# thomasdeppisch/eMagLS

Hardware: AMD Instinct MI355X
Metric: eMagLS filter sets/s (N=4, 2702 dirs, 512 taps) (higher is better)
Workload: dtype f64; 1 GPU; BASELINE config 3: getEMagLsFilters em32 r=4.2cm N=4 complex-SH, 2702 dirs, 512 taps, 48 kHz; one filter set per step, inputs resident in HBM; dirs=2702, taps=512, sim_order=19, bins=512, k_cut=43, designs_resident_per_gpu=128, designs_per_batch=32, batches_in_flight=4, distinct_hrir_sets_resident=20, parallelism=independent jobs per GPU, one RCCL gather

## Files before the change

### emagls_amd/csrc/fft.hip

```cpp
#include "kernels.hpp"
#include "lds_fft.hpp"
#include "wave_fft.hpp"

namespace emagls {

__global__ void twiddle_kernel(int nfft, cplx* __restrict__ tw, size_t bstride) {
    tw = boff(tw, bstride);
    int j = blockIdx.x * blockDim.x + threadIdx.x;
    if (j >= nfft) return;
    double s, c;
    sincos(-2.0 * kPi * (double)j / (double)nfft, &s, &c);
    if (j == 0) { c = 1.0; s = 0.0; }
    if (2 * j == nfft) { c = -1.0; s = 0.0; }
    if (4 * j == nfft) { c = 0.0; s = -1.0; }
    if (4 * j == 3 * nfft) { c = 0.0; s = 1.0; }
    tw[j] = mk(c, s);
}

__global__ void __launch_bounds__(256) hrir_dirsum_kernel(const double* __restrict__ hL, const double* __restrict__ hR,
                                                          int64_t L, int64_t D, int chunk, double* __restrict__ partial, size_t bstride) {
    hL = boff(hL, bstride); hR = boff(hR, bstride); partial = boff(partial, bstride);
    const int e = blockIdx.y;
    const double* h = e ? hR : hL;
    const int64_t d0 = (int64_t)blockIdx.x * chunk;
// ... 225 lines not shown
                double* row = Habs + ((int64_t)e * na + (kb - kabs0)) * ldD + d0;
                if (nt == HF_TD) {
#pragma unroll
                    for (int t = 0; t < HF_TD; t += 2) *reinterpret_cast<double2*>(row + t) = make_double2(habs[s][e][t], habs[s][e][t + 1]);
                } else {
#pragma unroll
                    for (int t = 0; t < HF_TD; ++t) if (t < nt) row[t] = habs[s][e][t];
                }
            }
        }
    }
}

constexpr int HW_TD = 8;
constexpr int HW_STRIDE = WF_BUF + 1;
__global__ void __launch_bounds__(64 * HW_TD) hrir_fft_wave_kernel(const double* __restrict__ hL, const double* __restrict__ hR,
                                                                   int64_t L, int64_t D, const int64_t* __restrict__ didx,
                                                                   const cplx* __restrict__ tw, const double* __restrict__ grpd,
                                                                   int mode, int n_c, int kabs0, cplx* __restrict__ Hc,
                                                                   double* __restrict__ Habs, int64_t ldD, double* __restrict__ HcT, int ldT,
                                                                   size_t bstride) {
    hL = boff(hL, bstride); hR = boff(hR, bstride); didx = boff(didx, bstride); tw = boff(tw, bstride); grpd = boff(grpd, bstride); Hc = boff(Hc, bstride); Habs = boff(Habs, bstride);
    HcT = boff(HcT, bstride);
    extern __shared__ __attribute__((aligned(16))) char smem[];
    constexpr int P = WF_N / 2 + 1;
    cplx* tables = reinterpret_cast<cplx*>(smem);
    cplx* bufs = tables + WF_TABLES;
    const int tid = threadIdx.x, w = tid >> 6, l = tid & 63;
    wave_fft_tables(tables, tw, tid, 64 * HW_TD);
    __syncthreads();
    const int64_t d0 = (int64_t)blockIdx.x * HW_TD;
    const int nt = (int)min((int64_t)HW_TD, D - d0);
    cplx* tb = bufs + (size_t)w * HW_STRIDE;
    if (w < nt) {
        const int64_t d = d0 + w;
        const int64_t dsrc = didx ? didx[d] : d;
        const double* pl = hL + dsrc * L;
        const double* pr = hR + dsrc * L;
        cplx v[16];
        const bool upper_zero = mode == 0 && L <= WF_N / 2;
        if (mode == 0) {
#pragma unroll
            for (int n1 = 0; n1 < 16; ++n1) {
                const int n = 64 * n1 + l;
                v[n1] = (n < L && (n1 < 8 || !upper_zero)) ? mk(pl[n], pr[n]) : mk(0.0, 0.0);
            }
        } else {
            const int sL = (int)round(grpd[0]), sR = (int)round(grpd[1]);
#pragma unroll
            for (int n1 = 0; n1 < 16; ++n1) {
                const int n = 64 * n1 + l;
                int nl = (n + sL) % WF_N; if (nl < 0) nl += WF_N;
                int nr = (n + sR) % WF_N; if (nr < 0) nr += WF_N;
                v[n1] = mk(nl < L ? pl[nl] : 0.0, nr < L ? pr[nr] : 0.0);
            }
        }
        bool nzL = false, nzR = false;
#pragma unroll
        for (int n1 = 0; n1 < 16; ++n1) { nzL |= v[n1].x != 0.0; nzR |= v[n1].y != 0.0; }
        const bool liveL = __any(nzL), liveR = __any(nzR);
        if (upper_zero) wave_fft1024<true>(v, tb, tables, l); else wave_fft1024<false>(v, tb, tables, l);
        wave_fft_store_natural(v, tb, l);
        wave_lds_fence();
        const cplx* phs = reinterpret_cast<const cplx*>(grpd + 2);
#pragma unroll
        for (int s = 0; s < 9; ++s) {
            const int kb = l + 64 * s;
            if (kb < P) {
                const cplx z = tb[wf_slot(kb)], zc = conj(tb[wf_slot((WF_N - kb) & (WF_N - 1))]);
                cplx HLv = mk(0.5 * (z.x + zc.x), 0.5 * (z.y + zc.y));
                cplx HRv = mk(0.5 * (z.y - zc.y), -0.5 * (z.x - zc.x));
                if (mode == 0) {
                    HLv = HLv * phs[kb];
                    HRv = HRv * phs[P + kb];
                }
                if (!liveL) HLv = mk(0.0, 0.0);
                if (!liveR) HRv = mk(0.0, 0.0);
                if (kb < n_c) {
                    Hc[((int64_t)0 * n_c + kb) * ldD + d] = HLv;
                    Hc[((int64_t)1 * n_c + kb) * ldD + d] = HRv;
                    if (HcT) {
                        double* rowT = HcT + d * ldT;
                        *reinterpret_cast<cplx*>(rowT + 2 * kb) = HLv;
                        *reinterpret_cast<cplx*>(rowT + 2 * (n_c + kb)) = HRv;
                    }
                }
                const double nl2 = norm2(HLv), nr2 = norm2(HRv);
                tb[wf_slot(kb)] = mk(nl2 > 0.0 ? nl2 * fast_rsqrt(nl2) : 0.0, nr2 > 0.0 ? nr2 * fast_rsqrt(nr2) : 0.0);
            }
        }
    }
    __syncthreads();
    const int64_t na = P - kabs0;
    const int t = tid & (HW_TD - 1);
    if (t < nt) {
        const double* src = reinterpret_cast<const double*>(bufs + (size_t)t * HW_STRIDE);
        for (int idx = tid >> 3; idx < 2 * (P - kabs0); idx += 64) {
            const int e = idx >= P - kabs0, kr = idx - e * (P - kabs0);
            Habs[((int64_t)e * na + kr) * ldD + d0 + t] = src[2 * wf_slot(kr + kabs0) + e];
        }
    }
}

__global__ void __launch_bounds__(512) real_fft_gather_kernel(const double* __restrict__ x, int64_t L, int64_t ncols,
                                                              const int64_t* __restrict__ colidx, int nfft, int log2n,
                                                              int TP, const cplx* __restrict__ tw,
                                                              cplx* __restrict__ out, int64_t ldo, int64_t inner,
                                                              int64_t ld_inner) {
    extern __shared__ __attribute__((aligned(16))) char smem[];
    cplx* tws = reinterpret_cast<cplx*>(smem);
    cplx* buf = tws + nfft / 2;
    const int P = nfft / 2 + 1;
    const int64_t p0 = (int64_t)blockIdx.x * TP;
    const int64_t npairs = (ncols + 1) / 2;
    const int nt = (int)min((int64_t)TP, npairs - p0);
// ... 270 lines not shown
                     int64_t ldD, hipStream_t st, double* HcT, int ldT) {
    if (!is_pow2(nfft)) {
        int td = HD_TD;
        while (td > 1 && (size_t)td * 2 * L * 8 > 48 * 1024) td >>= 1;
        if ((size_t)td * 2 * L * 8 > 64 * 1024) throw Error(2, "HRIR DFT: more than 4096 taps is not supported");
        hrir_dft_kernel<<<bgrid((unsigned)ceil_div(D, td)), 256, (size_t)td * 2 * L * 8, st>>>(hL, hR, L, D, didx, nfft, (const cplx*)tw, grpd, mode, n_c, kabs0,
                                                                                                (cplx*)Hc, Habs, ldD, HcT, ldT, td, batch_ctx().stride);
        KERNEL_CHECK();
        return;
    }
    const int log2n = ilog2(nfft);
    const int P = nfft / 2 + 1;
    if (P > HF_MAXS * 512) throw Error(2, "HRIR FFT: nfft above 2048 is not supported");
    if (nfft == WF_N && L <= WF_N && sw_on<Sw::HRIR_FFT_WAVE>()) {
        const size_t smw = sizeof(cplx) * (WF_TABLES + (size_t)HW_TD * HW_STRIDE);
        static PerDeviceOnce wave_once;
        if (wave_once.first())
            HIP_CHECK(hipFuncSetAttribute((const void*)hrir_fft_wave_kernel, hipFuncAttributeMaxDynamicSharedMemorySize, 160 * 1024));
        hrir_fft_wave_kernel<<<bgrid((unsigned)ceil_div(D, HW_TD)), 64 * HW_TD, smw, st>>>(hL, hR, L, D, didx, (const cplx*)tw, grpd, mode, n_c, kabs0,
                                                                                      (cplx*)Hc, Habs, ldD, HcT, ldT, batch_ctx().stride);
        KERNEL_CHECK();
        return;
    }
    size_t budget = (nfft >= 2048 ? 110 : 83) * 1024;
    if (const int kb = sw_int<Sw::HRIR_FFT_LDS_KB>()) budget = (size_t)kb * 1024;
    const size_t shared = (size_t)2 * P * 16 + 2 * HF_TD * sizeof(int);
    int TS = HF_TD;
    while (TS > 1 && (size_t)TS * nfft * 16 + shared > budget) TS >>= 1;
    const size_t sm = (size_t)TS * nfft * 16 + shared;
    static PerDeviceOnce attr_once;
    if (attr_once.first()) {
        HIP_CHECK(hipFuncSetAttribute((const void*)hrir_fft_kernel<8>, hipFuncAttributeMaxDynamicSharedMemorySize, 160 * 1024));
        HIP_CHECK(hipFuncSetAttribute((const void*)hrir_fft_kernel<4>, hipFuncAttributeMaxDynamicSharedMemorySize, 160 * 1024));
        HIP_CHECK(hipFuncSetAttribute((const void*)hrir_fft_kernel<2>, hipFuncAttributeMaxDynamicSharedMemorySize, 160 * 1024));
        HIP_CHECK(hipFuncSetAttribute((const void*)hrir_fft_kernel<1>, hipFuncAttributeMaxDynamicSharedMemorySize, 160 * 1024));
// ... 64 lines not shown
```

### emagls_amd/csrc/sweep_reg.hip

```cpp
#include "device_mem.hpp"
#include "persist_common.hpp"
#include "synth_common.hpp"

#include <algorithm>
#include <map>
#include <mutex>

namespace emagls {

namespace {

constexpr int RG_MLD = 36;

constexpr int DPP_ROR4 = 0x124, DPP_ROR8 = 0x128;
__device__ __forceinline__ int rg_slot_set(int i, int x) { return i < 4 ? 0 : i < 8 ? 1 : x >> 1; }
__device__ __forceinline__ int rg_slot_unit(int i, int x) { return i < 8 ? 4 * (i & 3) + x : 16 + (x & 1); }

template <int NUL>
__device__ __forceinline__ void rg_contract(const cplx (&E)[NUL], const cplx (&O)[NUL], const cplx (&ts)[2], int lane, bool slot8, double* wp) {
    static_assert(NUL == 9, "quad layout of 18 units");
    const int x = lane & 3;
    double ar[2], ai[2];
#pragma unroll
    for (int s = 0; s < 2; ++s) { ar[s] = (x & 1) ? ts[s].y : ts[s].x; ai[s] = (x & 1) ? -ts[s].x : ts[s].y; }
// ... 70 lines not shown
        if (n + 2 >= nord_pad) break;
        request(n + 4, b0, b1);
        pass(c0, c1);
        lds_wait2(b0, b1, pb[GS - 1]);
    }
}

__device__ __forceinline__ int launder(int v) { asm volatile("" : "+v"(v)); return v; }

#define RG_GLOBAL(T, p) ((T __attribute__((address_space(1)))*)(p))
typedef const double __attribute__((address_space(1)))* gcd_t;
typedef const cplx __attribute__((address_space(1)))* gcc_t;
typedef u64 __attribute__((address_space(1)))* gu64_t;
typedef unsigned u32x4_t __attribute__((ext_vector_type(4)));
__device__ __forceinline__ cplx ldg(gcc_t p) { return mk(p->x, p->y); }
__device__ __forceinline__ u64 gll_load(gu64_t p) { return __hip_atomic_load(p, __ATOMIC_RELAXED, __HIP_MEMORY_SCOPE_AGENT); }
__device__ __forceinline__ void gll_put(gu64_t dst, u64 word, bool local) {
    if (local) __hip_atomic_store(dst, word, __ATOMIC_RELAXED, __HIP_MEMORY_SCOPE_WORKGROUP);
    else __hip_atomic_store(dst, word, __ATOMIC_RELAXED, __HIP_MEMORY_SCOPE_AGENT);
}
__device__ __forceinline__ void gll_load16_async(u32x4_t& out, gu64_t p) { asm volatile("global_load_dwordx4 %0, %1, off sc1" : "=v"(out) : "v"(p) : "memory"); }

constexpr int RG_POLL = 12;
__device__ __forceinline__ void rg_wait_loads(u32x4_t (&g)[RG_POLL]) {
    asm volatile("s_waitcnt vmcnt(0)" : "+v"(g[0]), "+v"(g[1]), "+v"(g[2]), "+v"(g[3]), "+v"(g[4]), "+v"(g[5]), "+v"(g[6]), "+v"(g[7]), "+v"(g[8]), "+v"(g[9]),
                 "+v"(g[10]), "+v"(g[11]) :: "memory");
}
constexpr int RG_NUL = 9;
constexpr int RG_NEX = 4 * PS_CMAX;
constexpr int RG_SVC = 256;

template <int NUL, int NW>
__global__ void __launch_bounds__(64 * NW) __attribute__((amdgpu_waves_per_eu(3))) sweep_reg_kernel(const HalfSweepArgs* __restrict__ args, int n, int nWG, int spread, int prio) {
    constexpr int NT = 64 * NW, DPW = 32 * NW;
    constexpr int NU2 = 2 * NUL;
    constexpr int NVW = 8 * NU2;
    constexpr int GA = (NUL + 1) / 2, GB = NUL - GA;
    static_assert(GB >= 1 && NW % 2 == 0 && NT >= RG_SVC, "layout");
    extern __shared__ __attribute__((aligned(16))) char dyn[];
    cplx* ring = reinterpret_cast<cplx*>(dyn);
    cplx* ms = ring + 2 * SY_NORD;
    cplx* WE = ms + PS_CMAX * RG_MLD;
    cplx* WO = WE + 2 * NU2;
    double* vt = reinterpret_cast<double*>(WO + 2 * NU2);
    double* wpart = vt + 2 * RG_NEX;
    double* xs = wpart + NW * NVW;
    __shared__ int s_abort, s_local;

    int design, member;
    if (spread) {
        design = (int)blockIdx.x / nWG;
        member = (int)blockIdx.x - design * nWG;
    } else {
        const int xcd = blockIdx.x & 7, rest = blockIdx.x >> 3;
        const int sub = rest / nWG;
        member = rest - sub * nWG;
        design = xcd + 8 * sub;
    }
    if (design >= n) return;
    if (prio) __builtin_amdgcn_s_setprio(3);
    const HalfSweepArgs& a = args[design];
    const int tid = threadIdx.x;
    const int C = a.C, P = a.P, D = a.D, kfirst = a.kfirst, kabs0 = a.kabs0;
    const int64_t ldH = a.ldH;
    const int nord_pad = a.nord_pad;
    const gcd_t Habs = RG_GLOBAL(const double, a.Habs);
    const gcc_t Mw = RG_GLOBAL(const cplx, a.Mw);
    const gcc_t bsc = RG_GLOBAL(const cplx, a.bsc);
    const gcd_t Winit = RG_GLOBAL(const double, a.Winit);
    cplx __attribute__((address_space(1)))* const Uout = RG_GLOBAL(cplx, a.U);
    long long* const timing = a.timing;
    int* const abort_flag = a.abort_flag;
    const long long wait_ticks = a.wait_ticks;
    const int* smap = a.smap;
    const int npr = smap[32], nsg = smap[33], nun = npr + nsg;
    const gu64_t part_ll = RG_GLOBAL(u64, a.ll);
    const gu64_t xcc_ll = part_ll + (size_t)2 * nWG * RG_NEX * 2;
    if (tid == 0) { s_abort = 0; s_local = 0; }
    const int d0 = member * DPW;
// ... 20 lines not shown
                synth_zen(a.mic_zen ? a.mic_zen[jm] : 1.5707963267948966, sm, cm);
                v = synth_x2(s ? sd[1] : sd[0], s ? cd[1] : cd[0], sm, cm, (s ? daz[1] : daz[0]) - a.mic_azi[jm]);
            }
            xs[i * NT + tid] = v;
        }
    }
    __syncthreads();

    if (tid < nord_pad) {
        ring[(kfirst & 1) * SY_NORD + tid] = ldg(bsc + (int64_t)kfirst * nord_pad + tid);
        const int k1 = kfirst + 1 < P ? kfirst + 1 : P - 1;
        ring[((kfirst + 1) & 1) * SY_NORD + tid] = ldg(bsc + (int64_t)k1 * nord_pad + tid);
    }
    constexpr int NLM = 4;
    cplx mReg[NLM];
    auto fetch_m = [&](int kbm, int t) __attribute__((always_inline)) {
        const int r = t >> 3, c0 = (t & 7) * 4;
        const gcc_t M = Mw + (int64_t)kbm * C * C + r * C + c0;
#pragma unroll
        for (int i = 0; i < NLM; ++i) mReg[i] = ldg(M + i);
    };
    auto stage_m = [&](int t) __attribute__((always_inline)) {
        const int r = t >> 3, c0 = (t & 7) * 4;
#pragma unroll
        for (int i = 0; i < NLM; ++i) ms[r * RG_MLD + c0 + i] = (r < C && c0 + i < C) ? mReg[i] : mk(0, 0);
    };
    double hCur[2], hNext[2] = {0.0, 0.0};
    auto fetch_h = [&](int kb, double (&h)[2], int t) __attribute__((always_inline)) {
        const int kbg = (kb < P ? kb : P - 1) - kabs0;
        const gcd_t He = Habs + ((int64_t)((t >> 1) & 1) * (P - kabs0) + kbg) * ldH;
#pragma unroll
        for (int s = 0; s < 2; ++s) h[s] = He[dir_of(t, s) < D ? dir_of(t, s) : D - 1];
    };
    fetch_h(kfirst, hCur, tid);
    if (tid < RG_SVC) { fetch_m(kfirst, tid); stage_m(tid); }

    if (tid < 64) {
        const int lane = tid;
        const unsigned xcc = read_xcc_id();
        const unsigned tag0 = 0x58434300u;
        if (lane == 0) gll_put(xcc_ll + member, ((u64)tag0 << 32) | xcc, false);
        bool alive = true, same = true;
        for (int base = 0; base < nWG && alive; base += 64) {
            u64 w = 0;
            alive = ll_wait([&] {
                if (base + lane >= nWG) return true;
                w = gll_load(xcc_ll + base + lane);
                return ll_ok(w, tag0);
            }, abort_flag, wait_ticks);
            same = same && __builtin_amdgcn_ballot_w64(base + lane < nWG && (unsigned)w != xcc) == 0;
// ... 24 lines not shown
            const double* xcol = xs + launder(tid);
            synth_units<0, GA, NUL, NT>(xcol, E, O, bs, nord_pad);
            __builtin_amdgcn_sched_barrier(0);
            if (slot8) synth_units<GA, GB, NUL, NT>(xcol, E, O, bs, nord_pad);
            else synth_units<GA, GB - 1, NUL, NT>(xcol, E, O, bs, nord_pad);
            __builtin_amdgcn_sched_barrier(0);
        }
        RSTAMP(0);
        if (launder(tid) < RG_SVC) {
            const int t = launder(tid);
            const int j = t & (RG_NEX - 1), half = t >> 7;
            if (first) {
                vt[t] = half == 0 ? Winit[j] : 0.0;
            } else {
                const unsigned tag = (unsigned)(kb - 1);
                const gu64_t src = part_ll + ((size_t)((kb - 1) & 1) * nWG * RG_NEX + j) * 2;
                double sum = 0.0;
                const bool alive = ll_wait([&] {
                    bool ok = true;
                    double s = 0.0;
                    for (int base = half; base < nWG; base += 2 * RG_POLL) {
                        u32x4_t g[RG_POLL];
#pragma unroll
                        for (int i = 0; i < RG_POLL; ++i) {
                            const int w = base + 2 * i < nWG ? base + 2 * i : half;
                            gll_load16_async(g[i], src + (size_t)w * RG_NEX * 2);
                        }
                        rg_wait_loads(g);
#pragma unroll
                        for (int i = 0; i < RG_POLL; ++i) {
                            ok = ok && g[i].y == tag && g[i].w == tag;
                            if (base + 2 * i < nWG) s += __hiloint2double((int)g[i].z, (int)g[i].x);
                        }
                    }
                    sum = s;
                    return ok;
                }, abort_flag, wait_ticks);
                vt[t] = sum;
                if (!alive && (t & 63) == 0) s_abort = 1;
            }
        }
// ... 2 lines not shown
        if (s_abort) break;
        if (launder(tid) < RG_SVC) {
            const int t = launder(tid);
            const int part = t & 3, pair = t >> 2, e = pair >> 5, c = pair & 31;
            const cplx* vc = reinterpret_cast<const cplx*>(vt) + e * PS_CMAX;
            cplx acc = mk(0, 0);
            if (first) {
                if (part == 0) acc = vc[c];
            } else {
#pragma unroll
                for (int i = 0; i < PS_CMAX / 4; ++i)
                    cfma(acc, vc[part + 4 * i] + vc[RG_NEX / 2 + part + 4 * i], conj(ms[(part + 4 * i) * RG_MLD + c]));
            }
            acc = group_sum<4>(acc);
            const cplx other = shfl_xor_c(acc, 4);
            if (part == 0 && c < C) {
                if (c < 2 * npr) {
                    if ((c & 1) == 0) { WE[e * NU2 + (c >> 1)] = acc + other; WO[e * NU2 + (c >> 1)] = acc - other; }
                } else {
                    WE[e * NU2 + npr + (c - 2 * npr)] = acc; WO[e * NU2 + npr + (c - 2 * npr)] = acc;
                }
                if (member == 0 && !first) {
                    cplx __attribute__((address_space(1)))* dst = Uout + ((int64_t)e * P + (kb - 1)) * PS_CMAX + c;
                    const cplx v = vc[c] + vc[RG_NEX / 2 + c];
                    dst->x = v.x; dst->y = v.y;
                }
            }
        }
        if (last) break;
        __syncthreads();
        RSTAMP(3);
        const bool svc = launder(tid) < RG_SVC;
        if (svc) fetch_m(kb, launder(tid));
        cplx ts[2];
        {
            const int t = launder(tid);
            const int x = t & 3;
            cplx p[2][2];
#pragma unroll
            for (int s = 0; s < 2; ++s) { p[s][0] = mk(0, 0); p[s][1] = mk(0, 0); }
#pragma unroll
            for (int r = 0; r < 4; ++r) {
                const int u = 4 * r + x;
                const cplx we0 = WE[u], wo0 = WO[u], we1 = WE[NU2 + u], wo1 = WO[NU2 + u];
#pragma unroll
                for (int s = 0; s < 2; ++s) {
                    cfma(p[s][0], we0, E[4 * s + r]); cfma(p[s][0], wo0, O[4 * s + r]);
                    cfma(p[s][1], we1, E[4 * s + r]); cfma(p[s][1], wo1, O[4 * s + r]);
                }
            }
            if (slot8) {
                const int u = 16 + (x & 1);
                cplx q0 = mk(0, 0), q1 = mk(0, 0);
                cfma(q0, WE[u], E[8]); cfma(q0, WO[u], O[8]);
                cfma(q1, WE[NU2 + u], E[8]); cfma(q1, WO[NU2 + u], O[8]);
                const bool s1 = (x & 2) != 0;
                const cplx z = mk(0, 0);
                p[0][0] = p[0][0] + (s1 ? z : q0); p[0][1] = p[0][1] + (s1 ? z : q1);
                p[1][0] = p[1][0] + (s1 ? q0 : z); p[1][1] = p[1][1] + (s1 ? q1 : z);
            }
            if (svc) stage_m(t);
            RSTAMP(8);
#pragma unroll
            for (int s = 0; s < 2; ++s) {
                const cplx pe0 = group_sum<4>(p[s][0]), pe1 = group_sum<4>(p[s][1]);
                const cplx pe = (x & 2) ? pe1 : pe0;
                ts[s] = dir_of(t, s) < D ? unit_phase(hCur[s], pe, nyq) : mk(0, 0);
            }
        }
        __builtin_amdgcn_sched_barrier(0);
        {
            const int t = launder(tid);
            rg_contract<NUL>(E, O, ts, t & 63, slot8, wpart + (t >> 6) * NVW);
        }
        {
            const int t = launder(tid);
            fetch_h(kb + 1, hNext, t);
            if (t < nord_pad) ring[(kb & 1) * SY_NORD + t] = ldg(bsc + (int64_t)(kb + 2 < P ? kb + 2 : P - 1) * nord_pad + t);
        }
        __syncthreads();
        RSTAMP(4);
        if (launder(tid) < RG_NEX) {
            const int t = launder(tid);
            const int xe = t >> 6, xr = (t >> 1) & 31, xri = t & 1;
            double v = 0.0;
            if (xr < C) {
                const int xu = xr < 2 * npr ? (xr >> 1) : npr + (xr - 2 * npr);
                const bool xneg = xr < 2 * npr && (xr & 1);
                const double* wE = wpart + 8 * xu + 2 * xe + xri;
                double sE = 0.0, sO = 0.0;
#pragma unroll
                for (int w = 0; w < NW; ++w) { sE += wE[w * NVW]; sO += wE[w * NVW + 4]; }
                v = xneg ? sE - sO : sE + sO;
            }
            const gu64_t dst = part_ll + (((size_t)(kb & 1) * nWG + member) * RG_NEX + t) * 2;
            const u64 bits = (u64)__double_as_longlong(v), tg = (u64)(unsigned)kb << 32;
            gll_put(dst, tg | (bits & 0xffffffffull), local);
            gll_put(dst + 1, tg | (bits >> 32), local);
        }
        RSTAMP(5);
        hCur[0] = hNext[0]; hCur[1] = hNext[1];
    }
#undef RSTAMP
}

__global__ void __launch_bounds__(64) reg_contract_selftest_kernel(const cplx* __restrict__ t, const cplx* __restrict__ g, double* __restrict__ out) {
    const int lane = threadIdx.x, x = lane & 3;
    cplx E[RG_NUL], O[RG_NUL], ts[2];
#pragma unroll
    for (int i = 0; i < RG_NUL; ++i) {
// ... 160 lines not shown
```

### emagls_amd/csrc/switches.hpp

```cpp
#pragma once
#include <climits>
#include <cmath>

namespace emagls {

#define EMAGLS_SWITCHES(X) \
    X(PLAN_CACHE,        INT,  4,     0, INT_MAX,   PROCESS, "shapes the one-shot entry points keep alive (0 = off)") \
    X(BATCH_MAX,         INT,  8,     1, 32,        PROCESS, "initial limit of designs per batch, read at load time (emagls_set_batch_max changes it at run time; the job scheduler sets it per chunk)") \
    X(BATCH_GROUPS,      INT,  2,     1, 4,         CALL,    "lane groups of a batch of more than 8 designs before its sweep (1 = one launch sequence)") \
    X(BATCH_LANES,       ON0,  1,     0, 1,         CALL,    "=0: batches in stream mode (per-plan pipelines) instead of lane mode") \
    X(DEBUG_LANES,       ON1,  0,     0, 1,         CALL,    "=1: why a batch was refused lane mode or common routes, on stderr") \
    X(STAGGER,           ON0,  1,     0, 1,         PROCESS, "=0: both lane groups of a batch issue the stages before the sweep in one order (default: complementary orders)") \
    X(DEFER_HH,          INT,  1,     0, 2,         PROCESS, "the orthonormal route of the low bins next to the sweep: 0 never, 1 batches and designs that have the device to themselves, 2 every lane batch") \
    X(GEO_KEEP,          ON0,  1,     0, 1,         PROCESS, "=0: sharing batches run their geometry stages on every execute") \
    X(GRAM_LDS,          ON0,  1,     0, 1,         PROCESS, "=0: lane batches take the K-split Gram kernel + reduce instead of the LDS-staged one") \
    X(GRAM_MFMA4,        ON1,  0,     0, 1,         CALL,    "=1: the Gram tile on the 4 x 4 x 4 MFMA shape (measured slower; the tests' second form)") \
    X(XCD_RUNS,          ON0,  1,     0, 1,         PROCESS, "=0: gram_lds, gemm_tn_f64, synth_ls take their tiles in dispatch order instead of XCD-aware runs") \
    X(GRAM_ROUTE,        ON0,  1,     0, 1,         CALL,    "=0: no Gram route (all bins Householder + Jacobi)") \
    X(GRAM_COND_EST,     REAL, 3e3,   -HUGE_VAL, HUGE_VAL, CALL, "conditioning estimate below which the Gram route starts (the device check stays at 3e4)") \
    X(JACOBI_RUN,        INT,  0,     1, INT_MAX,   PROCESS, "bins per Jacobi workgroup on the Gram route (0: single bins where the stages are forked, runs of 2 in lane groups)") \
    X(REAL_INTERNAL,     ON0,  1,     0, 1,         CALL,    "=0: complex-basis eMagLS / eMagLS2 designs on the complex-arithmetic pipeline") \
    X(NO_GRAPH,          ON1,  0,     0, 1,         CALL,    "=1: eager launches instead of hipGraph replay (plans and batches, when they are created)") \
    X(STREAMS,           INT,  0,     1, 4,         CALL,    "streams of a single plan (0: one, until emagls_plan_set_streams)") \
    X(ONESHOT_STREAMS,   INT,  1,     1, 3,         CALL,    "streams of the one-shot plans of array designs") \
// ... 9 lines not shown
    X(SWEEP_WAIT_MS,     INT,  20,    1, INT_MAX,   PROCESS, "wall-clock limit of a wait for peers inside a resident sweep, in ms") \
    X(SWEEP_TIMING,      ON1,  0,     0, 1,         CALL,    "=1: in-kernel wall-clock stamps of the persistent sweep (when a plan is created)") \
    X(CU_BUDGET,         INT,  0,     0, INT_MAX,   CALL,    "CUs the resident sweeps may count on when their residency is decided (0: the device's)") \
    X(SYNTH_PAIRS,       ON0,  1,     0, 1,         PROCESS, "=0: synthesising sweep without antipodal microphone pairs") \
    X(SYNTH_SPLIT,       INT,  67,    INT_MIN, INT_MAX, PROCESS, "synthesising sweep: per cent of the producers' unit groups evaluated before barrier B1") \
    X(SYNTH_PRIO,        INT,  5,     0, 5,         PROCESS, "synthesising sweep: issue priorities (5: the chains of the two designs of an XCD tilted against the age order; 0: all chains 3, producers 0)") \
    X(STREAM_POOL,       ON0,  1,     0, 1,         PROCESS, "=0: destroy streams instead of recycling them (exposes a HIP runtime crash in long sessions)") \
    X(STREAM_WARM,       INT,  8,     0, INT_MAX,   PROCESS, "streams the pool parks before it hands the first one out") \
    X(POOL_GB,           INT,  128,   0, INT_MAX,   PROCESS, "device memory the block pool keeps for the next plans and arenas, in GB") \
    X(JOBS_FORK,         INT,  3,     1, 4,         PROCESS, "job scheduler: streams of a job list that is a single chunk (1 = lane groups as for chunks in flight)") \
    X(JOBS_RESIDENT,     INT,  0,     0, INT_MAX,   CALL,    "job scheduler: designs whose plans and batches stay resident between calls (0: max(256, 2 x batch x in flight))") \
    X(JOBS_AUTO_SHARE,   ON0,  1,     0, 1,         PROCESS, "=0: job scheduler shares no geometry unless the caller asks") \
    X(JOBS_TRACE,        ON1,  0,     0, 1,         PROCESS, "=1: time stamps of every chunk's steps and of block pool misses on stderr") \
    X(HRIR_FFT_WAVE,     ON0,  1,     0, 1,         CALL,    "=0: the HRIR prologue at nfft = 1024 on the LDS radix-2^2 transform instead of wave-private transforms") \
    X(HRIR_FFT_LDS_KB,   INT,  0,     40, 158,      CALL,    "LDS budget of the LDS-form HRIR transform's sub-tiles (0: 83, 110 at nfft = 2048)") \
    X(DECODE_FUSED,      ON0,  1,     0, 1,         CALL,    "=0: binauralDecode on the hipFFT passes for every filter length") \
    X(DECODE_REGFFT,     ON0,  1,     0, 1,         CALL,    "=0: the fused decode kernel on LDS transform passes also up to 512 taps") \
    X(DECODE_WAVE,       ON0,  1,     0, 1,         CALL,    "=0: the half-wave two-factor decode form also at 257-512 taps") \
    X(DECODE_FILTER_FFT, ONH,  0,     0, 1,         CALL,    "=hipfft: the filter side of the decode's wave form through hipFFT") \
    X(WA_REG,            ON0,  1,     0, 1,         CALL,    "=0: the 33-64-channel path's Householder kernels walk the columns through L2") \
    X(WA_TALL,           ON0,  1,     0, 1,         CALL,    "=0: the plain Householder kernels for problems of more than 448 rows instead of the LDS-reflector forms") \
    X(WA_YRI_MFMA,       ON0,  1,     0, 1,         CALL,    "=0: the 33-64-channel path's Y_reg_inv_k product on the vector pipe") \
    X(WA_JACOBI_FLAG,    REAL, 1e-14, -HUGE_VAL, HUGE_VAL, PROCESS, "the 33-64-channel path's Jacobi: another sweep follows one in which some rotation had |gamma| > x sqrt(alpha beta)") \
    X(WA_LEAF_ROWS,      INT,  0,     INT_MIN, INT_MAX, PROCESS, "tiled QR: upper bound of the leaf height, 1024 .. 4096 (anything else: 3072)")

enum class Sw : int {
#define X(name, kind, def, lo, hi, when, doc) name,
    EMAGLS_SWITCHES(X)
#undef X
    COUNT
// ... 22 lines not shown
```

### emagls_amd/csrc/wave_fft.hpp

```cpp
#pragma once
#include "reg_fft.hpp"

namespace emagls {

constexpr int WF_N = 1024;
constexpr int WF_ROW = 68;
constexpr int WF_BUF = 16 * WF_ROW;
constexpr int WF_TW1 = 1024;
constexpr int WF_TW2 = 64;
constexpr int WF_TABLES = WF_TW1 + WF_TW2;

__host__ __device__ constexpr int wf_bin(int l, int i) { return (l >> 2) + 16 * ((l & 3) + 4 * (i >> 3)) + 128 * rf_bitrev<3>(i & 7); }
__host__ __device__ constexpr int wf_slot(int k) { return (k & ~7) | ((k + 2 * ((k >> 4) & 3)) & 7); }

__device__ __forceinline__ void wave_fft_tables(cplx* tables, const cplx* __restrict__ circle, int tid, int nthreads) {
    for (int idx = tid; idx < WF_TW1; idx += nthreads) tables[idx] = circle[(idx & 63) * rf_bitrev<4>(idx >> 6)];
    for (int idx = tid; idx < WF_TW2; idx += nthreads) {
        const int d = idx >> 5, j = (idx >> 2) & 7, s = idx & 3;
        tables[WF_TW1 + idx] = circle[16 * ((s + 4 * d) * rf_bitrev<3>(j))];
    }
}

__device__ __forceinline__ void wave_lds_fence() {
    __builtin_amdgcn_fence(__ATOMIC_RELEASE, "wavefront");
// ... 10 lines not shown
    for (int i = 0; i < 8; ++i) {
        const cplx a = v[i];
        if (i == 0) v[8] = a;
        else if (i == 4) v[12] = mk(a.y, -a.x);
        else v[8 + i] = mk(a.x * C16[i] - a.y * S16[i], a.x * S16[i] + a.y * C16[i]);
    }
    cplx lo[8], hi[8];
#pragma unroll
    for (int i = 0; i < 8; ++i) { lo[i] = v[i]; hi[i] = v[8 + i]; }
    reg_fft<8>(lo);
    reg_fft<8>(hi);
#pragma unroll
    for (int i = 0; i < 8; ++i) { v[i] = lo[i]; v[8 + i] = hi[i]; }
}

template <bool UPPER_ZERO>
__device__ __forceinline__ void wf_pass1(cplx (&v)[16], cplx* tb, const cplx* tables, int l) {
    if (UPPER_ZERO) reg_fft16_upper_zero(v); else reg_fft<16>(v);
    const int lsw = (l & ~7) | ((l + (l >> 3)) & 7);
#pragma unroll
    for (int i0 = 0; i0 < 16; i0 += 4) {
        cplx t[4];
#pragma unroll
        for (int i = 0; i < 4; ++i) t[i] = tables[(i0 + i) * 64 + l];
#pragma unroll
        for (int i = 0; i < 4; ++i) tb[rf_bitrev<4>(i0 + i) * WF_ROW + lsw] = v[i0 + i] * t[i];
        __builtin_amdgcn_sched_barrier(0);
    }
    wave_lds_fence();
}
template <int H>
__device__ __forceinline__ void wf_pass2_half(cplx* tb, const cplx* tables, int l) {
    const int b = (l & 3) + 4 * H;
    cplx* row = tb + (l >> 2) * WF_ROW;
    const cplx* tw2 = tables + WF_TW1 + 32 * H + (l & 3);
    cplx u[8];
#pragma unroll
    for (int a = 0; a < 8; ++a) u[a] = row[8 * a + ((b + a) & 7)];
    reg_fft<8>(u);
#pragma unroll
    for (int j = 0; j < 8; ++j) {
        const int ka = rf_bitrev<3>(j);
        row[8 * ka + ((b + ka) & 7)] = (j == 0) ? u[j] : u[j] * tw2[4 * j];
    }
}
template <int E>
__device__ __forceinline__ void wf_pass3_half(cplx (&out)[8], const cplx* tb, int l) {
    const int ka = (l & 3) + 4 * E;
    const cplx* rowk = tb + (l >> 2) * WF_ROW + 8 * ka;
#pragma unroll
    for (int b = 0; b < 8; ++b) out[b] = rowk[(b + ka) & 7];
    reg_fft<8>(out);
}

template <bool UPPER_ZERO>
__device__ __forceinline__ void wave_fft1024(cplx (&v)[16], cplx* tb, const cplx* tables, int l) {
    wf_pass1<UPPER_ZERO>(v, tb, tables, l);
    wf_pass2_half<0>(tb, tables, l);
    wf_pass2_half<1>(tb, tables, l);
    wave_lds_fence();
    cplx u0[8], u1[8];
    wf_pass3_half<0>(u0, tb, l);
    wf_pass3_half<1>(u1, tb, l);
    wave_lds_fence();
#pragma unroll
    for (int j = 0; j < 8; ++j) { v[j] = u0[j]; v[8 + j] = u1[j]; }
}

__device__ __forceinline__ void wave_fft_store_natural(const cplx (&v)[16], cplx* tb, int l) {
    const int base = (l >> 2) + 16 * (l & 3);
#pragma unroll
    for (int i = 0; i < 16; ++i) tb[wf_slot(base + 64 * (i >> 3) + 128 * rf_bitrev<3>(i & 7))] = v[i];
}

}
```

Measured before the change: 3913 filter sets/s.

## Make HRIR wave FFT persistent with prefetch and zero-row-pruned first pass

The HRIR wave-FFT kernel becomes a grid-stride persistent loop with a capped workgroup count. Each workgroup loads the next direction group's taps during the current FFT, so global loads overlap compute and the twiddle tables are built once per workgroup. The first radix-16 pass is specialised on the number of nonzero input rows (2/4/8/16, picked from the tap count), which cuts flops for short HRIRs. Separately, the sweep kernel switches to 32-bit offsets, uses wave-uniform pointer increments instead of per-bin recomputation, and issues the bsc row load early. These changes add register pressure, template variants and extra syncthreads per iteration.

```diff
diff --git a/emagls_amd/csrc/fft.hip b/emagls_amd/csrc/fft.hip
--- a/emagls_amd/csrc/fft.hip
+++ b/emagls_amd/csrc/fft.hip
@@ -263,91 +263,142 @@
 
 constexpr int HW_TD = 8;
 constexpr int HW_STRIDE = WF_BUF + 1;
+__device__ __forceinline__ int hw_launder(int v) { asm volatile("" : "+v"(v)); return v; }
+constexpr int HW_WALKERS = 1024;
+template <int NZ, bool SHIFT>
 __global__ void __launch_bounds__(64 * HW_TD) hrir_fft_wave_kernel(const double* __restrict__ hL, const double* __restrict__ hR,
                                                                    int64_t L, int64_t D, const int64_t* __restrict__ didx,
                                                                    const cplx* __restrict__ tw, const double* __restrict__ grpd,
-                                                                   int mode, int n_c, int kabs0, cplx* __restrict__ Hc,
+                                                                   int n_c, int kabs0, cplx* __restrict__ Hc,
                                                                    double* __restrict__ Habs, int64_t ldD, double* __restrict__ HcT, int ldT,
                                                                    size_t bstride) {
+    static_assert(!SHIFT || NZ == 16, "the circular shift reaches every input row");
+    const int64_t ngroups = (D + HW_TD - 1) / HW_TD;
+    if ((int64_t)blockIdx.x >= ngroups) return;
     hL = boff(hL, bstride); hR = boff(hR, bstride); didx = boff(didx, bstride); tw = boff(tw, bstride); grpd = boff(grpd, bstride); Hc = boff(Hc, bstride); Habs = boff(Habs, bstride);
     HcT = boff(HcT, bstride);
     extern __shared__ __attribute__((aligned(16))) char smem[];
     constexpr int P = WF_N / 2 + 1;
     cplx* tables = reinterpret_cast<cplx*>(smem);
     cplx* bufs = tables + WF_TABLES;
-    const int tid = threadIdx.x, w = tid >> 6, l = tid & 63;
-    wave_fft_tables(tables, tw, tid, 64 * HW_TD);
-    __syncthreads();
-    const int64_t d0 = (int64_t)blockIdx.x * HW_TD;
-    const int nt = (int)min((int64_t)HW_TD, D - d0);
-    cplx* tb = bufs + (size_t)w * HW_STRIDE;
-    if (w < nt) {
-        const int64_t d = d0 + w;
-        const int64_t dsrc = didx ? didx[d] : d;
-        const double* pl = hL + dsrc * L;
-        const double* pr = hR + dsrc * L;
-        cplx v[16];
-        const bool upper_zero = mode == 0 && L <= WF_N / 2;
-        if (mode == 0) {
-#pragma unroll
-            for (int n1 = 0; n1 < 16; ++n1) {
-                const int n = 64 * n1 + l;
-                v[n1] = (n < L && (n1 < 8 || !upper_zero)) ? mk(pl[n], pr[n]) : mk(0.0, 0.0);
-            }
-        } else {
-            const int sL = (int)round(grpd[0]), sR = (int)round(grpd[1]);
-#pragma unroll
-            for (int n1 = 0; n1 < 16; ++n1) {
-                const int n = 64 * n1 + l;
-                int nl = (n + sL) % WF_N; if (nl < 0) nl += WF_N;
-                int nr = (n + sR) % WF_N; if (nr < 0) nr += WF_N;
-                v[n1] = mk(nl < L ? pl[nl] : 0.0, nr < L ? pr[nr] : 0.0);
-            }
-        }
-        bool nzL = false, nzR = false;
-#pragma unroll
-        for (int n1 = 0; n1 < 16; ++n1) { nzL |= v[n1].x != 0.0; nzR |= v[n1].y != 0.0; }
-        const bool liveL = __any(nzL), liveR = __any(nzR);
-        if (upper_zero) wave_fft1024<true>(v, tb, tables, l); else wave_fft1024<false>(v, tb, tables, l);
-        wave_fft_store_natural(v, tb, l);
-        wave_lds_fence();
-        const cplx* phs = reinterpret_cast<const cplx*>(grpd + 2);
-#pragma unroll
-        for (int s = 0; s < 9; ++s) {
-            const int kb = l + 64 * s;
-            if (kb < P) {
-                const cplx z = tb[wf_slot(kb)], zc = conj(tb[wf_slot((WF_N - kb) & (WF_N - 1))]);
-                cplx HLv = mk(0.5 * (z.x + zc.x), 0.5 * (z.y + zc.y));
-                cplx HRv = mk(0.5 * (z.y - zc.y), -0.5 * (z.x - zc.x));
-                if (mode == 0) {
-                    HLv = HLv * phs[kb];
-                    HRv = HRv * phs[P + kb];
+    const int tid0 = threadIdx.x, w = tid0 >> 6;
+    wave_fft_tables(tables, tw, tid0, 64 * HW_TD);
+    const cplx* phs = reinterpret_cast<const cplx*>(grpd + 2);
+    int sL = 0, sR = 0;
+    if (SHIFT) { sL = (int)round(grpd[0]); sR = (int)round(grpd[1]); }
+    auto source_entry = [&](int64_t g) __attribute__((always_inline)) -> int64_t {
+        const int64_t d = g * HW_TD + w;
+        const int64_t dd = (g < ngroups && d < D) ? d : 0;
+        const int64_t* ip = didx ? didx + dd : reinterpret_cast<const int64_t*>(hL);
+        return *ip;
+    };
+    auto source_of = [&](int64_t g, int64_t entry) __attribute__((always_inline)) -> int64_t {
+        const int64_t d = g * HW_TD + w;
+        return (g < ngroups && d < D) ? (didx ? entry : d) : -1;
+    };
+    cplx v[16];
+    auto tap_index = [&](int n, int& nl, int& nr) __attribute__((always_inline)) {
+        nl = n; nr = n;
+        if (SHIFT) {
+            nl = (n + sL) % WF_N; if (nl < 0) nl += WF_N;
+            nr = (n + sR) % WF_N; if (nr < 0) nr += WF_N;
+        }
+    };
+    auto request = [&](int64_t dsrc) __attribute__((always_inline)) {
+        const int l = hw_launder(tid0) & 63;
+        const int64_t ds = dsrc >= 0 ? dsrc : 0;
+        const double* pl = hL + ds * L;
+        const double* pr = hR + ds * L;
+#pragma unroll
+        for (int n1 = 0; n1 < NZ; ++n1) {
+            int nl, nr;
+            tap_index(64 * n1 + l, nl, nr);
+            v[n1] = mk(pl[nl < L ? nl : 0], pr[nr < L ? nr : 0]);
+        }
+    };
+    auto taps_in = [&]() __attribute__((always_inline)) {
+        const int l = hw_launder(tid0) & 63;
+#pragma unroll
+        for (int n1 = 0; n1 < 16; ++n1) {
+            if (n1 >= NZ) { v[n1] = mk(0.0, 0.0); continue; }
+            int nl, nr;
+            tap_index(64 * n1 + l, nl, nr);
+            v[n1] = mk(nl < L ? v[n1].x : 0.0, nr < L ? v[n1].y : 0.0);
+        }
+    };
+    int64_t g = blockIdx.x;
+    int64_t entry_next = source_entry(g + gridDim.x);
+    request(source_of(g, source_entry(g)));
+    __syncthreads();
+    const int64_t na = P - kabs0;
+    for (; g < ngroups; g += gridDim.x) {
+        const int64_t d0 = g * HW_TD;
+        const int nt = (int)min((int64_t)HW_TD, D - d0);
+        if (w < nt) {
+            const int64_t d = d0 + w;
+            int l = hw_launder(tid0) & 63;
+            cplx* tb = bufs + (size_t)(hw_launder(tid0) >> 6) * HW_STRIDE;
+            taps_in();
+            bool nzL = false, nzR = false;
+#pragma unroll
+            for (int n1 = 0; n1 < NZ; ++n1) { nzL |= v[n1].x != 0.0; nzR |= v[n1].y != 0.0; }
+            const bool liveL = __any(nzL), liveR = __any(nzR);
+            cplx phL[9], phR[9];
+            if (!SHIFT) {
+#pragma unroll
+                for (int s = 0; s < 9; ++s) {
+                    const int kb = l + 64 * s < P ? l + 64 * s : P - 1;
+                    phL[s] = phs[kb]; phR[s] = phs[P + kb];
                 }
-                if (!liveL) HLv = mk(0.0, 0.0);
-                if (!liveR) HRv = mk(0.0, 0.0);
-                if (kb < n_c) {
-                    Hc[((int64_t)0 * n_c + kb) * ldD + d] = HLv;
-                    Hc[((int64_t)1 * n_c + kb) * ldD + d] = HRv;
-                    if (HcT) {
-                        double* rowT = HcT + d * ldT;
-                        *reinterpret_cast<cplx*>(rowT + 2 * kb) = HLv;
-                        *reinterpret_cast<cplx*>(rowT + 2 * (n_c + kb)) = HRv;
+            }
+            wf_pass1_nz<NZ>(v, tb, tables, l);
+            request(source_of(g + gridDim.x, entry_next));
+            entry_next = source_entry(g + 2 * (int64_t)gridDim.x);
+            l = hw_launder(tid0) & 63;
+            tb = bufs + (size_t)(hw_launder(tid0) >> 6) * HW_STRIDE;
+            cplx z16[16];
+            wave_fft1024_finish(z16, tb, tables, l);
+            wave_fft_store_natural(z16, tb, l);
+            wave_lds_fence();
+            l = hw_launder(tid0) & 63;
+            tb = bufs + (size_t)(hw_launder(tid0) >> 6) * HW_STRIDE;
+#pragma unroll
+            for (int s = 0; s < 9; ++s) {
+                const int kb = l + 64 * s;
+                if (kb < P) {
+                    const cplx z = tb[wf_slot(kb)], zc = conj(tb[wf_slot((WF_N - kb) & (WF_N - 1))]);
+                    cplx HLv = mk(0.5 * (z.x + zc.x), 0.5 * (z.y + zc.y));
+                    cplx HRv = mk(0.5 * (z.y - zc.y), -0.5 * (z.x - zc.x));
+                    if (!SHIFT) {
+                        HLv = HLv * phL[s];
+                        HRv = HRv * phR[s];
                     }
+                    if (!liveL) HLv = mk(0.0, 0.0);
+                    if (!liveR) HRv = mk(0.0, 0.0);
+                    if (kb < n_c) {
+                        Hc[((int64_t)0 * n_c + kb) * ldD + d] = HLv;
+                        Hc[((int64_t)1 * n_c + kb) * ldD + d] = HRv;
+                        if (HcT) {
+                            double* rowT = HcT + d * ldT;
+                            *reinterpret_cast<cplx*>(rowT + 2 * kb) = HLv;
+                            *reinterpret_cast<cplx*>(rowT + 2 * (n_c + kb)) = HRv;
+                        }
+                    }
+                    const double nl2 = norm2(HLv), nr2 = norm2(HRv);
+                    tb[wf_slot(kb)] = mk(nl2 > 0.0 ? nl2 * fast_rsqrt(nl2) : 0.0, nr2 > 0.0 ? nr2 * fast_rsqrt(nr2) : 0.0);
                 }
-                const double nl2 = norm2(HLv), nr2 = norm2(HRv);
-                tb[wf_slot(kb)] = mk(nl2 > 0.0 ? nl2 * fast_rsqrt(nl2) : 0.0, nr2 > 0.0 ? nr2 * fast_rsqrt(nr2) : 0.0);
-            }
-        }
-    }
-    __syncthreads();
-    const int64_t na = P - kabs0;
-    const int t = tid & (HW_TD - 1);
-    if (t < nt) {
-        const double* src = reinterpret_cast<const double*>(bufs + (size_t)t * HW_STRIDE);
-        for (int idx = tid >> 3; idx < 2 * (P - kabs0); idx += 64) {
-            const int e = idx >= P - kabs0, kr = idx - e * (P - kabs0);
-            Habs[((int64_t)e * na + kr) * ldD + d0 + t] = src[2 * wf_slot(kr + kabs0) + e];
-        }
+            }
+        }
+        __syncthreads();
+        const int tid = hw_launder(tid0), t = tid & (HW_TD - 1);
+        if (t < nt) {
+            const double* srcH = reinterpret_cast<const double*>(bufs + (size_t)t * HW_STRIDE);
+            for (int idx = tid >> 3; idx < 2 * (P - kabs0); idx += 64) {
+                const int e = idx >= P - kabs0, kr = idx - e * (P - kabs0);
+                Habs[((int64_t)e * na + kr) * ldD + d0 + t] = srcH[2 * wf_slot(kr + kabs0) + e];
+            }
+        }
+        __syncthreads();
     }
 }
 
@@ -648,11 +699,25 @@
     if (P > HF_MAXS * 512) throw Error(2, "HRIR FFT: nfft above 2048 is not supported");
     if (nfft == WF_N && L <= WF_N && sw_on<Sw::HRIR_FFT_WAVE>()) {
         const size_t smw = sizeof(cplx) * (WF_TABLES + (size_t)HW_TD * HW_STRIDE);
+        int wgs = (int)ceil_div(HW_WALKERS, std::max(batch_ctx().n, 1));
+        if (const int cap = sw_int<Sw::HRIR_FFT_WGS>()) wgs = std::min(wgs, cap);
+        const dim3 grid = bgrid((unsigned)std::min<int64_t>(ceil_div(D, HW_TD), wgs));
+        const int nz = mode != 0 ? 16 : L <= 128 ? 2 : L <= 256 ? 4 : L <= 512 ? 8 : 16;
         static PerDeviceOnce wave_once;
-        if (wave_once.first())
-            HIP_CHECK(hipFuncSetAttribute((const void*)hrir_fft_wave_kernel, hipFuncAttributeMaxDynamicSharedMemorySize, 160 * 1024));
-        hrir_fft_wave_kernel<<<bgrid((unsigned)ceil_div(D, HW_TD)), 64 * HW_TD, smw, st>>>(hL, hR, L, D, didx, (const cplx*)tw, grpd, mode, n_c, kabs0,
-                                                                                      (cplx*)Hc, Habs, ldD, HcT, ldT, batch_ctx().stride);
+#define EMAGLS_HW(NZV, SHV)                                                                                                             \
+    hrir_fft_wave_kernel<NZV, SHV><<<grid, 64 * HW_TD, smw, st>>>(hL, hR, L, D, didx, (const cplx*)tw, grpd, n_c, kabs0, (cplx*)Hc, Habs, \
+                                                                  ldD, HcT, ldT, batch_ctx().stride)
+#define EMAGLS_HW_LDS(NZV, SHV) HIP_CHECK(hipFuncSetAttribute((const void*)hrir_fft_wave_kernel<NZV, SHV>, hipFuncAttributeMaxDynamicSharedMemorySize, 160 * 1024))
+        if (wave_once.first()) { EMAGLS_HW_LDS(2, false); EMAGLS_HW_LDS(4, false); EMAGLS_HW_LDS(8, false); EMAGLS_HW_LDS(16, false); EMAGLS_HW_LDS(16, true); }
+        if (mode != 0) EMAGLS_HW(16, true);
+        else switch (nz) {
+            case 2: EMAGLS_HW(2, false); break;
+            case 4: EMAGLS_HW(4, false); break;
+            case 8: EMAGLS_HW(8, false); break;
+            default: EMAGLS_HW(16, false); break;
+        }
+#undef EMAGLS_HW_LDS
+#undef EMAGLS_HW
         KERNEL_CHECK();
         return;
     }
diff --git a/emagls_amd/csrc/sweep_reg.hip b/emagls_amd/csrc/sweep_reg.hip
--- a/emagls_amd/csrc/sweep_reg.hip
+++ b/emagls_amd/csrc/sweep_reg.hip
@@ -108,6 +108,12 @@
 typedef u64 __attribute__((address_space(1)))* gu64_t;
 typedef unsigned u32x4_t __attribute__((ext_vector_type(4)));
 __device__ __forceinline__ cplx ldg(gcc_t p) { return mk(p->x, p->y); }
+template <class T>
+__device__ __forceinline__ T __attribute__((address_space(1)))* rg_uniform(T __attribute__((address_space(1)))* p) {
+    const u64 v = (u64)p;
+    const u64 lo = (unsigned)__builtin_amdgcn_readfirstlane((int)(unsigned)v), hi = (unsigned)__builtin_amdgcn_readfirstlane((int)(unsigned)(v >> 32));
+    return (T __attribute__((address_space(1)))*)(lo | (hi << 32));
+}
 __device__ __forceinline__ u64 gll_load(gu64_t p) { return __hip_atomic_load(p, __ATOMIC_RELAXED, __HIP_MEMORY_SCOPE_AGENT); }
 __device__ __forceinline__ void gll_put(gu64_t dst, u64 word, bool local) {
     if (local) __hip_atomic_store(dst, word, __ATOMIC_RELAXED, __HIP_MEMORY_SCOPE_WORKGROUP);
@@ -131,6 +137,7 @@
     constexpr int NVW = 8 * NU2;
     constexpr int GA = (NUL + 1) / 2, GB = NUL - GA;
     static_assert(GB >= 1 && NW % 2 == 0 && NT >= RG_SVC, "layout");
+    constexpr bool ROW_EARLY = NT - RG_SVC >= SY_NORD;
     extern __shared__ __attribute__((aligned(16))) char dyn[];
     cplx* ring = reinterpret_cast<cplx*>(dyn);
     cplx* ms = ring + 2 * SY_NORD;
@@ -156,7 +163,7 @@
     const HalfSweepArgs& a = args[design];
     const int tid = threadIdx.x;
     const int C = a.C, P = a.P, D = a.D, kfirst = a.kfirst, kabs0 = a.kabs0;
-    const int64_t ldH = a.ldH;
+    const int ldH = (int)a.ldH;
     const int nord_pad = a.nord_pad;
     const gcd_t Habs = RG_GLOBAL(const double, a.Habs);
     const gcc_t Mw = RG_GLOBAL(const cplx, a.Mw);
@@ -207,26 +214,30 @@
     }
     constexpr int NLM = 4;
     cplx mReg[NLM];
-    auto fetch_m = [&](int kbm, int t) __attribute__((always_inline)) {
+    auto fetch_m = [&](gcc_t Mk, int t) __attribute__((always_inline)) {
         const int r = t >> 3, c0 = (t & 7) * 4;
-        const gcc_t M = Mw + (int64_t)kbm * C * C + r * C + c0;
+        const gcc_t M = Mk + (unsigned)(__mul24(r, C) + c0);
 #pragma unroll
         for (int i = 0; i < NLM; ++i) mReg[i] = ldg(M + i);
     };
     auto stage_m = [&](int t) __attribute__((always_inline)) {
         const int r = t >> 3, c0 = (t & 7) * 4;
 #pragma unroll
-        for (int i = 0; i < NLM; ++i) ms[r * RG_MLD + c0 + i] = (r < C && c0 + i < C) ? mReg[i] : mk(0, 0);
+        for (int i = 0; i < NLM; ++i) ms[__mul24(r, RG_MLD) + c0 + i] = (r < C && c0 + i < C) ? mReg[i] : mk(0, 0);
     };
     double hCur[2], hNext[2] = {0.0, 0.0};
-    auto fetch_h = [&](int kb, double (&h)[2], int t) __attribute__((always_inline)) {
-        const int kbg = (kb < P ? kb : P - 1) - kabs0;
-        const gcd_t He = Habs + ((int64_t)((t >> 1) & 1) * (P - kabs0) + kbg) * ldH;
-#pragma unroll
-        for (int s = 0; s < 2; ++s) h[s] = He[dir_of(t, s) < D ? dir_of(t, s) : D - 1];
+    auto fetch_h = [&](gcd_t H0, unsigned ear1, double (&h)[2], int t) __attribute__((always_inline)) {
+        const unsigned e = (t & 2) ? ear1 : 0u;
+#pragma unroll
+        for (int s = 0; s < 2; ++s) h[s] = H0[e + (unsigned)(dir_of(t, s) < D ? dir_of(t, s) : D - 1)];
     };
-    fetch_h(kfirst, hCur, tid);
-    if (tid < RG_SVC) { fetch_m(kfirst, tid); stage_m(tid); }
+    const unsigned hear = (unsigned)((P - kabs0) * ldH);
+    const auto bin_row = [&](int k) { return k < P ? k : P - 1; };
+    gcd_t hrow = rg_uniform(Habs + (bin_row(kfirst + 1) - kabs0) * ldH);
+    gcc_t brow = rg_uniform(bsc + bin_row(kfirst + 2) * nord_pad);
+    gcc_t mrow = rg_uniform(Mw + kfirst * C * C);
+    fetch_h(Habs + (bin_row(kfirst) - kabs0) * ldH, hear, hCur, tid);
+    if (tid < RG_SVC) { fetch_m(mrow, tid); stage_m(tid); }
 
     if (tid < 64) {
         const int lane = tid;
@@ -281,7 +292,7 @@
                 vt[t] = half == 0 ? Winit[j] : 0.0;
             } else {
                 const unsigned tag = (unsigned)(kb - 1);
-                const gu64_t src = part_ll + ((size_t)((kb - 1) & 1) * nWG * RG_NEX + j) * 2;
+                const gu64_t src = part_ll + (unsigned)((((kb - 1) & 1) * nWG * RG_NEX + j) * 2);
                 double sum = 0.0;
                 const bool alive = ll_wait([&] {
                     bool ok = true;
@@ -291,7 +302,7 @@
 #pragma unroll
                         for (int i = 0; i < RG_POLL; ++i) {
                             const int w = base + 2 * i < nWG ? base + 2 * i : half;
-                            gll_load16_async(g[i], src + (size_t)w * RG_NEX * 2);
+                            gll_load16_async(g[i], src + (unsigned)(w * (RG_NEX * 2)));
                         }
                         rg_wait_loads(g);
 #pragma unroll
@@ -324,14 +335,15 @@
             }
             acc = group_sum<4>(acc);
             const cplx other = shfl_xor_c(acc, 4);
+            const int eu = e ? NU2 : 0;
             if (part == 0 && c < C) {
                 if (c < 2 * npr) {
-                    if ((c & 1) == 0) { WE[e * NU2 + (c >> 1)] = acc + other; WO[e * NU2 + (c >> 1)] = acc - other; }
+                    if ((c & 1) == 0) { WE[eu + (c >> 1)] = acc + other; WO[eu + (c >> 1)] = acc - other; }
                 } else {
-                    WE[e * NU2 + npr + (c - 2 * npr)] = acc; WO[e * NU2 + npr + (c - 2 * npr)] = acc;
+                    WE[eu + npr + (c - 2 * npr)] = acc; WO[eu + npr + (c - 2 * npr)] = acc;
                 }
                 if (member == 0 && !first) {
-                    cplx __attribute__((address_space(1)))* dst = Uout + ((int64_t)e * P + (kb - 1)) * PS_CMAX + c;
+                    cplx __attribute__((address_space(1)))* dst = Uout + (unsigned)(((e ? P : 0) + (kb - 1)) * PS_CMAX + c);
                     const cplx v = vc[c] + vc[RG_NEX / 2 + c];
                     dst->x = v.x; dst->y = v.y;
                 }
@@ -341,7 +353,9 @@
         __syncthreads();
         RSTAMP(3);
         const bool svc = launder(tid) < RG_SVC;
-        if (svc) fetch_m(kb, launder(tid));
+        const bool rowl = ROW_EARLY && !svc && launder(tid) - RG_SVC < nord_pad;
+        if (svc) fetch_m(mrow, launder(tid));
+        else if (rowl) mReg[0] = ldg(brow + (launder(tid) - RG_SVC));
         cplx ts[2];
         {
             const int t = launder(tid);
@@ -370,6 +384,7 @@
                 p[1][0] = p[1][0] + (s1 ? q0 : z); p[1][1] = p[1][1] + (s1 ? q1 : z);
             }
             if (svc) stage_m(t);
+            else if (rowl) ring[(kb & 1) * SY_NORD + (t - RG_SVC)] = mReg[0];
             RSTAMP(8);
 #pragma unroll
             for (int s = 0; s < 2; ++s) {
@@ -381,13 +396,17 @@
         __builtin_amdgcn_sched_barrier(0);
         {
             const int t = launder(tid);
-            rg_contract<NUL>(E, O, ts, t & 63, slot8, wpart + (t >> 6) * NVW);
-        }
+            rg_contract<NUL>(E, O, ts, t & 63, slot8, wpart + __mul24(t >> 6, NVW));
+        }
+        RSTAMP(9);
         {
             const int t = launder(tid);
-            fetch_h(kb + 1, hNext, t);
-            if (t < nord_pad) ring[(kb & 1) * SY_NORD + t] = ldg(bsc + (int64_t)(kb + 2 < P ? kb + 2 : P - 1) * nord_pad + t);
-        }
+            fetch_h(hrow, hear, hNext, t);
+            if (!ROW_EARLY && t < nord_pad) ring[(kb & 1) * SY_NORD + t] = ldg(brow + t);
+        }
+        if (kb + 2 < P) hrow += ldH;
+        if (kb + 3 < P) brow += nord_pad;
+        mrow += C * C;
         __syncthreads();
         RSTAMP(4);
         if (launder(tid) < RG_NEX) {
@@ -403,7 +422,7 @@
                 for (int w = 0; w < NW; ++w) { sE += wE[w * NVW]; sO += wE[w * NVW + 4]; }
                 v = xneg ? sE - sO : sE + sO;
             }
-            const gu64_t dst = part_ll + (((size_t)(kb & 1) * nWG + member) * RG_NEX + t) * 2;
+            const gu64_t dst = part_ll + (unsigned)((((kb & 1) * nWG + member) * RG_NEX + t) * 2);
             const u64 bits = (u64)__double_as_longlong(v), tg = (u64)(unsigned)kb << 32;
             gll_put(dst, tg | (bits & 0xffffffffull), local);
             gll_put(dst + 1, tg | (bits >> 32), local);
diff --git a/emagls_amd/csrc/switches.hpp b/emagls_amd/csrc/switches.hpp
--- a/emagls_amd/csrc/switches.hpp
+++ b/emagls_amd/csrc/switches.hpp
@@ -47,6 +47,7 @@
     X(JOBS_TRACE,        ON1,  0,     0, 1,         PROCESS, "=1: time stamps of every chunk's steps and of block pool misses on stderr") \
     X(HRIR_FFT_WAVE,     ON0,  1,     0, 1,         CALL,    "=0: the HRIR prologue at nfft = 1024 on the LDS radix-2^2 transform instead of wave-private transforms") \
     X(HRIR_FFT_LDS_KB,   INT,  0,     40, 158,      CALL,    "LDS budget of the LDS-form HRIR transform's sub-tiles (0: 83, 110 at nfft = 2048)") \
+    X(HRIR_FFT_WGS,      INT,  0,     0, 1024,      CALL,    "upper limit of the workgroups per design of the wave-form HRIR transform, each walking its share of the groups of 8 directions (0: 1024 over the lanes of the launch)") \
     X(DECODE_FUSED,      ON0,  1,     0, 1,         CALL,    "=0: binauralDecode on the hipFFT passes for every filter length") \
     X(DECODE_REGFFT,     ON0,  1,     0, 1,         CALL,    "=0: the fused decode kernel on LDS transform passes also up to 512 taps") \
     X(DECODE_WAVE,       ON0,  1,     0, 1,         CALL,    "=0: the half-wave two-factor decode form also at 257-512 taps") \
diff --git a/emagls_amd/csrc/wave_fft.hpp b/emagls_amd/csrc/wave_fft.hpp
--- a/emagls_amd/csrc/wave_fft.hpp
+++ b/emagls_amd/csrc/wave_fft.hpp
@@ -48,9 +48,50 @@
     for (int i = 0; i < 8; ++i) { v[i] = lo[i]; v[8 + i] = hi[i]; }
 }
 
-template <bool UPPER_ZERO>
-__device__ __forceinline__ void wf_pass1(cplx (&v)[16], cplx* tb, const cplx* tables, int l) {
-    if (UPPER_ZERO) reg_fft16_upper_zero(v); else reg_fft<16>(v);
+template <int E> __device__ __forceinline__ cplx rf_mul_w16(cplx a) {
+    constexpr double C16[8] = {1.0, 0.9238795325112867, 0.7071067811865476, 0.38268343236508984, 0.0, -0.3826834323650897,
+                               -0.7071067811865475, -0.9238795325112867};
+    constexpr double S16[8] = {0.0, -0.3826834323650898, -0.7071067811865475, -0.9238795325112867, -1.0, -0.9238795325112867,
+                               -0.7071067811865476, -0.3826834323650899};
+    constexpr int e = E & 15;
+    if (e == 0) return a;
+    if (e == 4) return mk(a.y, -a.x);
+    if (e == 8) return mk(-a.x, -a.y);
+    if (e == 12) return mk(-a.y, a.x);
+    constexpr double c = e < 8 ? C16[e & 7] : -C16[e & 7], sn = e < 8 ? S16[e & 7] : -S16[e & 7];
+    return mk(a.x * c - a.y * sn, a.x * sn + a.y * c);
+}
+__device__ __forceinline__ void reg_fft16_four(cplx (&v)[16]) {
+    const cplx a0 = v[0], a1 = v[1], a2 = v[2], a3 = v[3];
+#define EMAGLS_WF_QUARTER(Q, RR)                                                                                            \
+    {                                                                                                                       \
+        cplx u[4] = {a0, rf_mul_w16<RR>(a1), rf_mul_w16<2 * RR>(a2), rf_mul_w16<3 * RR>(a3)};                               \
+        reg_fft<4>(u);                                                                                                      \
+        v[4 * Q] = u[0]; v[4 * Q + 1] = u[1]; v[4 * Q + 2] = u[2]; v[4 * Q + 3] = u[3];                                     \
+    }
+    EMAGLS_WF_QUARTER(0, 0) EMAGLS_WF_QUARTER(1, 2) EMAGLS_WF_QUARTER(2, 1) EMAGLS_WF_QUARTER(3, 3)
+#undef EMAGLS_WF_QUARTER
+}
+template <int I> __device__ __forceinline__ void reg_fft16_two_step(cplx (&v)[16], cplx a0, cplx a1) {
+    const cplx b = rf_mul_w16<rf_bitrev<4>(I)>(a1);
+    v[I] = mk(a0.x + b.x, a0.y + b.y);
+    if constexpr (I + 1 < 16) reg_fft16_two_step<I + 1>(v, a0, a1);
+}
+__device__ __forceinline__ void reg_fft16_two(cplx (&v)[16]) {
+    const cplx a0 = v[0], a1 = v[1];
+    reg_fft16_two_step<0>(v, a0, a1);
+}
+template <int NZ> __device__ __forceinline__ void reg_fft16_nz(cplx (&v)[16]) {
+    static_assert(NZ == 2 || NZ == 4 || NZ == 8 || NZ == 16, "nonzero input rows");
+    if constexpr (NZ == 2) reg_fft16_two(v);
+    else if constexpr (NZ == 4) reg_fft16_four(v);
+    else if constexpr (NZ == 8) reg_fft16_upper_zero(v);
+    else reg_fft<16>(v);
+}
+
+template <int NZ>
+__device__ __forceinline__ void wf_pass1_nz(cplx (&v)[16], cplx* tb, const cplx* tables, int l) {
+    reg_fft16_nz<NZ>(v);
     const int lsw = (l & ~7) | ((l + (l >> 3)) & 7);
 #pragma unroll
     for (int i0 = 0; i0 < 16; i0 += 4) {
@@ -62,6 +103,10 @@
         __builtin_amdgcn_sched_barrier(0);
     }
     wave_lds_fence();
+}
+template <bool UPPER_ZERO>
+__device__ __forceinline__ void wf_pass1(cplx (&v)[16], cplx* tb, const cplx* tables, int l) {
+    wf_pass1_nz<UPPER_ZERO ? 8 : 16>(v, tb, tables, l);
 }
 template <int H>
 __device__ __forceinline__ void wf_pass2_half(cplx* tb, const cplx* tables, int l) {
@@ -87,9 +132,7 @@
     reg_fft<8>(out);
 }
 
-template <bool UPPER_ZERO>
-__device__ __forceinline__ void wave_fft1024(cplx (&v)[16], cplx* tb, const cplx* tables, int l) {
-    wf_pass1<UPPER_ZERO>(v, tb, tables, l);
+__device__ __forceinline__ void wave_fft1024_finish(cplx (&v)[16], cplx* tb, const cplx* tables, int l) {
     wf_pass2_half<0>(tb, tables, l);
     wf_pass2_half<1>(tb, tables, l);
     wave_lds_fence();
@@ -100,6 +143,11 @@
 #pragma unroll
     for (int j = 0; j < 8; ++j) { v[j] = u0[j]; v[8 + j] = u1[j]; }
 }
+template <bool UPPER_ZERO>
+__device__ __forceinline__ void wave_fft1024(cplx (&v)[16], cplx* tb, const cplx* tables, int l) {
+    wf_pass1<UPPER_ZERO>(v, tb, tables, l);
+    wave_fft1024_finish(v, tb, tables, l);
+}
 
 __device__ __forceinline__ void wave_fft_store_natural(const cplx (&v)[16], cplx* tb, int l) {
     const int base = (l >> 2) + 16 * (l & 3);
```

New measurement: 3807 filter sets/s. 0.973x the previous value.
